# Easquel/WaveDM

Hardware: AMD Instinct MI355X
Metric: restored images/sec, raindrop 64x64 patches, 100-step DDIM (higher is better)
Workload: dtype bf16; 1 GPU; raindrop_wavelet 64x64 (256x256 px crops), batch 64/GPU, 100 DDIM steps, DWT + UNet x100 + IDWT (BASELINE.json configs[1]); global_batch=64, ddim_steps=100, parallelism=image-sharded x1, outputs_finite=True

## Files before the change

wavedm_amd/csrc/attn.hip:

```cpp
#include <atomic>
#include <type_traits>

#include "common.h"
#include "attn_fused_kernel.h"

namespace wdm {

bool attn_fused_eligible(int dtype, int N, int C) {
    return env_cfg().attn_fused && is_h16(dtype) && N == AttnFusedCfg::N && C % 128 == 0 && C >= 128 && C <= AttnFusedCfg::MAX_C &&
           (C <= AttnFusedCfg::MAX_CP || (C / 2) % 128 == 0);
}

template <typename T, bool VTOK>
static int launch_attn_fused_t(const AttnOperands& in, void* o, int B, int C, hipStream_t s, const float* vbias, const ConvArgs* proj) {
    using Cf = AttnFusedCfg;
    const bool qproj = in.qw != nullptr;
    if ((!in.q && !qproj) || !in.k || !in.v || (!o && !proj) || B <= 0) WDM_FAIL(WDM_EINVAL, "attn(fused): bad argument");
    if (qproj && (!VTOK || !proj || in.q || in.k != in.v || in.qw_ld < C || in.qw_ld % 8 || in.qw_bytes == 0 || in.qw_bytes >= 4294901760.0))
        WDM_FAIL(WDM_EINVAL, "attn(fused): the in-kernel query projection needs the folded block's operands (K = V = the normalised input, proj_out fused)");
    if ((!qproj && in.q_ld < C) || in.k_ld < C || ((qproj ? 0 : in.q_ld) | in.k_ld) % 8 || (VTOK && (in.v_ld < C || in.v_ld % 8))) WDM_FAIL(WDM_EINVAL, "attn(fused): row strides must be multiples of 8 elements >= C");
    if (proj && (C > 512 || proj->Cout != C || proj->Cin != C || proj->Hout != 16 || proj->Wout != 16 || proj->B != B || !proj->w || proj->w_bytes == 0 || proj->y_mode != Y_NHWC ||
                 proj->temb || proj->m_valid || proj->up4 || (proj->stats && proj->stats_nslab != 4)))
        WDM_FAIL(WDM_EINVAL, "attn(fused): proj_out epilogue arguments do not describe a C = %d 1x1 conv on 16 x 16 maps", C);
    if (in.bdiag && (!VTOK || proj || qproj)) WDM_FAIL(WDM_EINVAL, "attn(fused): the block-diagonal form (64 tokens per image) takes token-major V and writes O");
    const int NT = in.bdiag ? 64 : Cf::N;
    const int G = in.bdiag ? (B + 3) / 4 : B;
    const double qb = (double)B * NT * in.q_ld * 2.0, kb = (double)B * NT * in.k_ld * 2.0, vb = VTOK ? (double)B * NT * in.v_ld * 2.0 : (double)B * C * Cf::N * 2.0;
    if (qb >= 4294901760.0 || kb >= 4294901760.0 || vb >= 4294901760.0) WDM_FAIL(WDM_EINVAL, "attn(fused): an operand exceeds the 4 GB buffer-offset range");
    AttnFusedArgs a{};
    a.q = in.q; a.k = in.k; a.v = in.v; a.o = o; a.vbias = vbias; a.B = G; a.C = C; a.bdiag = in.bdiag; a.nimg = B;
    a.q_ld = in.q_ld; a.k_ld = in.k_ld; a.v_ld = in.v_ld;
    a.alpha = (float)std::pow((double)C, -0.5);
    a.qw = in.qw; a.qbias = in.qbias; a.qw_ld = in.qw_ld; a.qw_bytes = (unsigned)in.qw_bytes; a.qw_slab = in.qw_slab;
    a.q_bytes = qproj ? 0u : (unsigned)(qb - (in.q_ld - C) * 2.0); a.k_bytes = (unsigned)(kb - (in.k_ld - C) * 2.0); a.v_bytes = (unsigned)(VTOK ? vb - (in.v_ld - C) * 2.0 : vb);
    static std::atomic<unsigned> devs{0};
    int dev = 0;
    WDM_HIP(hipGetDevice(&dev));
    if (!(devs.load() & (1u << (dev & 31)))) {
        WDM_HIP(hipFuncSetAttribute((const void*)attn_fused_kernel<false, T, VTOK>, hipFuncAttributeMaxDynamicSharedMemorySize, Cf::LDS_BYTES));
        WDM_HIP(hipFuncSetAttribute((const void*)attn_fused_kernel<true, T, VTOK>, hipFuncAttributeMaxDynamicSharedMemorySize, 160 * 1024));
        if constexpr (VTOK) WDM_HIP(hipFuncSetAttribute((const void*)attn_fused_kernel<true, T, true, true>, hipFuncAttributeMaxDynamicSharedMemorySize, 160 * 1024));
        devs.fetch_or(1u << (dev & 31));
    }
    const bool prof = prof_enabled();
    if (prof) {
        char name[96];
        snprintf(name, sizeof(name), "attn_fused_n%s%s%s_%s|%s C=%d%s%s", in.bdiag ? "64x4" : "256", VTOK ? "t" : "", qproj ? "q" : "", std::is_same<T, f16_t>::value ? "f16" : "bf16",
                 in.bdiag ? "8x8" : "16x16", C, qproj ? " qproj+" : "", proj ? " +proj" : "");
        prof_begin(s, name, 4.0 * B * NT * (double)NT * C + (proj ? 2.0 * B * Cf::N * (double)C * C : 0.0) + (qproj ? 2.0 * B * Cf::N * (double)C * C : 0.0),
                   (double)B * NT * C * 2.0 * (qproj ? 3.0 : proj ? 5.0 : 4.0) + (proj ? (double)C * C * 2.0 : 0.0) + (qproj ? (double)C * C * 2.0 : 0.0));
    }
    ConvArgs pe{};
    if (proj) pe = *proj;
// ... 16 lines not shown
```

wavedm_amd/csrc/attn_fused_kernel.h:

```cpp
#pragma once
#include "conv_kernel.h"
#include "gn_arrive.h"

namespace wdm {

struct AttnFusedArgs {
    const void* q;
    const void* k;
    const void* v;
    void* o;
    const float* vbias;
    int B, C;
    int q_ld, k_ld, v_ld;
    float alpha;
    unsigned q_bytes, k_bytes, v_bytes;
    const void* qw;
    const float* qbias;
    int qw_ld;
    unsigned qw_bytes;
    int qw_slab;
    int bdiag, nimg;
};

struct AttnFusedCfg {
// ... 27 lines not shown
    typedef int i32x4 __attribute__((ext_vector_type(4)));
    auto make_q = [](const void* p, unsigned bytes) __attribute__((always_inline)) {
        const unsigned long long v = (unsigned long long)p;
        return i32x4{(int)(unsigned)v, (int)((unsigned)(v >> 32) & 0xFFFFu), (int)bytes, 0x00020000};
    };
    const i32x4 q_q = make_q(a.q, a.q_bytes), q_k = make_q(a.k, a.k_bytes), q_vt = make_q(a.v, a.v_bytes);
    const unsigned lds0 = (unsigned)(size_t)(__attribute__((address_space(3))) char*)smem;
    auto dma16 = [&](const i32x4& rsrc, unsigned lds_addr, unsigned voff, int soff) __attribute__((always_inline)) {
        unsigned keep;
        asm volatile("s_mov_b32 %0, m0\n\ts_mov_b32 m0, %2\n\ts_nop 0\n\tbuffer_load_dwordx4 %1, %3, %4 offen lds\n\ts_mov_b32 m0, %0"
                     : "=&s"(keep)
                     : "v"(voff), "s"(lds_addr), "s"(rsrc), "s"(soff)
                     : "memory");
    };

    unsigned v1[5];
#pragma unroll
    for (int j = 0; j < 5; ++j) {
        const int piece = wave * 5 + j;
        const int row = piece * 8 + (lane >> 3);
        const int u = (lane & 7) ^ ((row >> 1) & 7);
        const bool isk = row < N;
        const int tok = isk ? row : qb * QB + (row - N);
        v1[j] = (unsigned)(((long long)b * N + tok) * (isk ? a.k_ld : a.q_ld) * 2 + u * 16);
    }
    constexpr int ST1Q = N * 128;
    constexpr int Q_OFF = 3 * ST1Q;
    if constexpr (QPROJ) {
#pragma unroll
        for (int j = 0; j < 4; ++j) {
            const int row = (wave * 4 + j) * 8 + (lane >> 3);
            const int u = (lane & 7) ^ ((row >> 1) & 7);
            v1[j] = (unsigned)(((long long)b * N + row) * a.k_ld * 2 + u * 16);
        }
    }
    auto issue1 = [&](int step, int buf) __attribute__((always_inline)) {
        if constexpr (QPROJ) {
            const unsigned base = lds0 + buf * ST1Q + wave * (4 * 1024);
#pragma unroll
            for (int j = 0; j < 4; ++j) dma16(q_k, base + j * 1024, v1[j], step * 128);
        } else {
        const unsigned base = lds0 + buf * C::ST1 + wave * (5 * 1024);
#pragma unroll
        for (int j = 0; j < 5; ++j) dma16(wave * 5 + j < N / 8 ? q_k : q_q, base + j * 1024, v1[j], step * 128);
        }
    };
    const int npass = Cc > C::MAX_CP ? 2 : 1;
// ... 19 lines not shown
    }
    auto issue2 = [&](int pass, int chunk, int buf) __attribute__((always_inline)) {
        const unsigned base = lds0 + C::P_BYTES + buf * C::ST2 + wave * (4 * 1024);
        const int soff = VTOK ? (chunk * 32 * a.v_ld + pass * Cp) * 2 : pass * Cp * N * 2 + chunk * 64;
#pragma unroll
        for (int j = 0; j < 4; ++j) dma16(q_vt, base + j * 1024, v2[j], soff);
    };

    const int wm = wave >> 1, wn = wave & 1;
    const int sw = (lane >> 1) & 7, ku = lane >> 4;
    int a_off[2], b_off[2];
#pragma unroll
    for (int ks = 0; ks < 2; ++ks) {
        const int slot = (ks * 4 + ku) ^ sw;
        a_off[ks] = (wm * 64 + (lane & 15)) * 128 + slot * 16;
        b_off[ks] = N * 128 + (wn * 32 + (lane & 15)) * 128 + slot * 16;
    }
    f32x4 s_acc[4][2];
#pragma unroll
    for (int i = 0; i < 4; ++i)
#pragma unroll
        for (int j = 0; j < 2; ++j) s_acc[i][j] = f32x4{0.f, 0.f, 0.f, 0.f};
    const int nk = Cc / 64;
    if constexpr (QPROJ) {
        constexpr int HQ_BYTES = QB * 512 * 2, ST0 = 512 * 64;
        static_assert(HQ_BYTES + 3 * ST0 <= 160 * 1024 && Q_OFF + QB * 512 * 2 <= 160 * 1024, "LDS");
        const i32x4 q_mw = make_q(a.qw, a.qw_bytes);
        const int np0 = Cc / 32;
#pragma unroll
        for (int j = 0; j < 8; ++j) {
            const int piece = wave * 8 + j;
            const int pl = piece >> 2, row = (piece & 3) * 16 + (lane >> 2);
            if (pl < np0) dma16(q_k, lds0 + piece * 1024, (unsigned)(((long long)b * N + qb * QB + row) * a.k_ld * 2 + un2 * 16), pl * 64);
        }
        unsigned v0[4];
#pragma unroll
        for (int j = 0; j < 4; ++j) {
            const int row = (wave * 4 + j) * 16 + (lane >> 2);
            v0[j] = row < Cc ? (unsigned)((a.qw_slab ? row * 32 : row * a.qw_ld) * 2 + un2 * 16) : 0xFFFF0000u;
        }
        const int qstep = a.qw_slab ? a.qw_slab * 2 : 64;
        auto issue0 = [&](int chunk, int buf) __attribute__((always_inline)) {
            const unsigned base = lds0 + HQ_BYTES + buf * ST0 + wave * (4 * 1024);
#pragma unroll
            for (int j = 0; j < 4; ++j) dma16(q_mw, base + j * 1024, v0[j], chunk * qstep);
        };
// ... 40 lines not shown
            const int plane = c0 >> 6, unit = (c0 & 63) >> 3, half = (c0 >> 2) & 1;
#pragma unroll
            for (int i = 0; i < 4; ++i) {
                const int qn = i * 16 + (lane & 15);
                const uint2 qv = make_uint2(TI<T>::pack2(__builtin_fmaf(y_acc[i][j][0], 1.0f, cb.x), __builtin_fmaf(y_acc[i][j][1], 1.0f, cb.y)),
                                            TI<T>::pack2(__builtin_fmaf(y_acc[i][j][2], 1.0f, cb.z), __builtin_fmaf(y_acc[i][j][3], 1.0f, cb.w)));
                if (c0 < Cc) *(uint2*)(smem + Q_OFF + plane * (QB * 128) + qn * 128 + ((unit ^ ((qn >> 1) & 7)) << 4) + half * 8) = qv;
            }
        }
    } else {
    issue1(0, 0);
    if (nk > 1) issue1(1, 1);
    }
    {
        int buf = 0;
        for (int k = 0; k < nk; ++k) {
            if (k + 1 < nk) { if constexpr (QPROJ) asm volatile("s_waitcnt vmcnt(4) lgkmcnt(0)" ::: "memory"); else asm volatile("s_waitcnt vmcnt(5) lgkmcnt(0)" ::: "memory"); }
            else asm volatile("s_waitcnt vmcnt(0) lgkmcnt(0)" ::: "memory");
            __builtin_amdgcn_s_barrier();
            __builtin_amdgcn_sched_barrier(0);
            if (k + 2 < nk) issue1(k + 2, buf >= 1 ? buf - 1 : 2);
            const char* base = smem + buf * (QPROJ ? ST1Q : C::ST1);
            const char* qbase = QPROJ ? smem + Q_OFF + k * (QB * 128) - N * 128 : base;
#pragma unroll
            for (int ks = 0; ks < 2; ++ks) {
                uint4 af[4], bf[2];
#pragma unroll
                for (int i = 0; i < 4; ++i) af[i] = *(const uint4*)(base + a_off[ks] + i * (16 * 128));
#pragma unroll
                for (int j = 0; j < 2; ++j) bf[j] = *(const uint4*)(qbase + b_off[ks] + j * (16 * 128));
#pragma unroll
                for (int i = 0; i < 4; ++i)
#pragma unroll
                    for (int j = 0; j < 2; ++j) mma16<T>(s_acc[i][j], af[i], bf[j]);
            }
            buf = buf == 2 ? 0 : buf + 1;
        }
    }
    asm volatile("s_waitcnt vmcnt(0) lgkmcnt(0)" ::: "memory");
    __builtin_amdgcn_s_barrier();
    __builtin_amdgcn_sched_barrier(0);
    issue2(0, 0, 0);
    issue2(0, 1, 1);

    float* red = (float*)(smem + C::RED_OFF);
    const float sl2 = a.alpha * 1.4426950408889634f;
    float mx[2], sm[2];
#pragma unroll
    for (int j = 0; j < 2; ++j) {
        float m = -INFINITY;
#pragma unroll
        for (int i = 0; i < 4; ++i)
#pragma unroll
            for (int r = 0; r < 4; ++r) { s_acc[i][j][r] = (a.bdiag && wm != qb) ? -INFINITY : s_acc[i][j][r] * sl2; m = fmaxf(m, s_acc[i][j][r]); }
        m = fmaxf(m, __shfl_xor(m, 16));
        m = fmaxf(m, __shfl_xor(m, 32));
        if (lane < 16) red[wm * QB + wn * 32 + j * 16 + lane] = m;
        mx[j] = m;
    }
    asm volatile("s_waitcnt lgkmcnt(0)" ::: "memory");
    __builtin_amdgcn_s_barrier();
    __builtin_amdgcn_sched_barrier(0);
#pragma unroll
    for (int j = 0; j < 2; ++j) {
        const int qn = wn * 32 + j * 16 + (lane & 15);
        const float m = fmaxf(fmaxf(red[qn], red[QB + qn]), fmaxf(red[2 * QB + qn], red[3 * QB + qn]));
// ... 25 lines not shown
    }
    (void)mx; (void)sm;

    const int cw = Cp / 8;
    const int nfi = cw / 16;
    const int va_off = C::P_BYTES + lds_off(wave * cw + (lane & 15), ku);
    unsigned va_tr[4];
#pragma unroll
    for (int i = 0; i < 4; ++i) {
        const int li = lane & 15, g = lane >> 4, bs = wave * (cw >> 4) + i;
        const int fr = (li >> 2) + 4 * (g & 1);
        va_tr[i] = lds0 + C::P_BYTES + (g * 8 + (li >> 2)) * rowb + ((bs & ~7) | ((bs + fr) & 7)) * 32 + (li & 3) * 8;
    }
    int pb_off[4];
#pragma unroll
    for (int j = 0; j < 4; ++j) pb_off[j] = (j * 16 + (lane & 15)) * 512;
    const int prow15 = lane & 15;
    T* op = (T*)a.o + ((long long)b * N + qb * QB) * Cc;
    for (int pass = 0; pass < npass; ++pass) {
        if (pass > 0) {
            asm volatile("s_waitcnt lgkmcnt(0)" ::: "memory");
            __builtin_amdgcn_s_barrier();
            __builtin_amdgcn_sched_barrier(0);
            issue2(pass, 0, 0);
            issue2(pass, 1, 1);
        }
        f32x4 o_acc[4][4];
#pragma unroll
        for (int i = 0; i < 4; ++i)
#pragma unroll
            for (int j = 0; j < 4; ++j) o_acc[i][j] = f32x4{0.f, 0.f, 0.f, 0.f};
        int buf = 0;
        for (int k = 0; k < N / 32; ++k) {
            if (k + 1 < N / 32) asm volatile("s_waitcnt vmcnt(4) lgkmcnt(0)" ::: "memory");
            else asm volatile("s_waitcnt vmcnt(0) lgkmcnt(0)" ::: "memory");
            if (k == 0 || !own_rows || VTOK) __builtin_amdgcn_s_barrier();
            __builtin_amdgcn_sched_barrier(0);
            if (k + 2 < N / 32) issue2(pass, k + 2, buf >= 1 ? buf - 1 : 2);
            const char* vb = smem + buf * C::ST2;
            uint4 af[4], bf[4];
            const int pslot = ((k * 4 + ku) ^ prow15) << 4;
            if constexpr (VTOK) {
                unsigned long long lo[4], hi[4];
                const unsigned sb = buf * C::ST2;
#pragma unroll
                for (int i = 0; i < 4; ++i) {
                    const unsigned ad = (i < nfi ? va_tr[i] : va_tr[0]) + sb;
                    asm volatile("ds_read_b64_tr_b16 %0, %1" : "=v"(lo[i]) : "v"(ad) : "memory");
                    asm volatile("ds_read_b64_tr_b16 %0, %1" : "=v"(hi[i]) : "v"(ad + 4 * rowb) : "memory");
                }
#pragma unroll
                for (int j = 0; j < 4; ++j) bf[j] = *(const uint4*)(smem + pb_off[j] + pslot);
                asm volatile("s_waitcnt lgkmcnt(0)" : "+v"(lo[0]), "+v"(lo[1]), "+v"(lo[2]), "+v"(lo[3]), "+v"(hi[0]), "+v"(hi[1]), "+v"(hi[2]), "+v"(hi[3]) :: "memory");
#pragma unroll
                for (int i = 0; i < 4; ++i) af[i] = uint4{(unsigned)lo[i], (unsigned)(lo[i] >> 32), (unsigned)hi[i], (unsigned)(hi[i] >> 32)};
            } else {
#pragma unroll
                for (int i = 0; i < 4; ++i) if (i < nfi) af[i] = *(const uint4*)(vb + va_off + i * (16 * 64));
#pragma unroll
                for (int j = 0; j < 4; ++j) bf[j] = *(const uint4*)(smem + pb_off[j] + pslot);
            }
// ... 84 lines not shown
```

wavedm_amd/csrc/blocks.hip:

```cpp
#include <stdarg.h>

#include <algorithm>
#include <cmath>

#include <atomic>
#include <mutex>
#include "common.h"
#include "gn_inline.h"

namespace wdm {

static thread_local char g_err[512] = "";
void set_error(const char* fmt, ...) {
    va_list ap;
    va_start(ap, fmt);
    vsnprintf(g_err, sizeof(g_err), fmt, ap);
    va_end(ap);
}
const char* get_error() { return g_err; }

void* Arena::alloc(size_t bytes) {
    bytes = align_up(bytes ? bytes : 1, 256);
    for (size_t i = 0; i < free_.size(); ++i) {
        if (free_[i].len >= bytes) {
// ... 32 lines not shown
    if (!t->p) WDM_FAIL(WDM_ENOMEM, "workspace too small (tensor %dx%dx%dx%d)", c.B, H, W, C);
    return WDM_OK;
}
void free_tens(Ctx& c, Tens& t) {
    c.ar->free(t.p);
    if (t.stats) c.ar->free(t.stats);
    if (t.nrm) c.ar->free(t.nrm);
    if (t.fin_scale) { c.ar->free(t.fin_scale); c.ar->free(t.fin_shift); }
    t.p = nullptr; t.stats = nullptr; t.gst = nullptr; t.nslab = 0; t.nrm = nullptr; t.nrm_for = nullptr; t.fin_scale = t.fin_shift = nullptr; t.fin_for = nullptr;
}

static int alloc_f32(Ctx& c, size_t n, float** p) {
    *p = (float*)c.ar->alloc(n * sizeof(float));
    if (!*p) WDM_FAIL(WDM_ENOMEM, "workspace too small (%zu floats)", n);
    return WDM_OK;
}

static std::atomic<const EnvCfg*> g_env{nullptr};
static std::mutex g_env_mu;
void env_cfg_refresh() {
    EnvCfg* c = new EnvCfg();
    auto flag = [](const char* name, int dflt) { const char* e = getenv(name); return e ? (e[0] == '0' ? 0 : 1) : dflt; };
    auto num = [](const char* name, int dflt) { const char* e = getenv(name); return e ? atoi(e) : dflt; };
    c->conv_dma = flag("WDM_CONV_DMA", 1); c->gemm = flag("WDM_GEMM", 1); c->bn256 = num("WDM_BN256", 1);
    c->gn_tile = num("WDM_GN_TILE", 2); c->gn_inline = num("WDM_GN_INLINE", 1); c->attn_fused = num("WDM_ATTN_FUSED", 3); c->attn_fold = num("WDM_ATTN_FOLD", 1);
    c->up4 = flag("WDM_UP4", 1); c->attn_sm = flag("WDM_ATTN_SM", 1); c->wgrad_bg = num("WDM_WGRAD_BG", 0);
    std::lock_guard<std::mutex> lk(g_env_mu);
    g_env.store(c, std::memory_order_release);
}
const EnvCfg& env_cfg() {
    const EnvCfg* c = g_env.load(std::memory_order_acquire);
    if (!c) {
        {
            std::lock_guard<std::mutex> lk(g_env_mu);
            c = g_env.load(std::memory_order_acquire);
        }
        if (!c) { env_cfg_refresh(); c = g_env.load(std::memory_order_acquire); }
    }
    return *c;
}

bool conv_up4_eligible(int dtype, int H, int W, int cin, int cout) {
    return env_cfg().up4 && (is_h16(dtype) || dtype == WDM_F32X3) && ((H % 16 == 0 && W % 16 == 0) || (H == 8 && W == 8)) && cin % 32 == 0 && cout % 8 == 0 && cout >= 128;
}

int launch_conv(const ConvArgs& a0, int mode, int dtype, hipStream_t s) {
    const ConvArgs& a = a0;
    return dtype == WDM_BF16 ? launch_conv_bf16(a, mode, s) : dtype == WDM_F16 ? launch_conv_f16(a, mode, s) : dtype == WDM_F32X3 ? launch_conv_f32x3(a, mode, s) : launch_conv_f32(a, mode, s);
// ... 351 lines not shown
```

wavedm_amd/csrc/common.h:

```cpp
#pragma once
#include <hip/hip_runtime.h>
#include <stdint.h>
#include <stdio.h>
#include <string>
#include <vector>

#include "../../include/wavedm.h"
#include "conv_kernel.h"

namespace wdm {

void set_error(const char* fmt, ...);
#define WDM_FAIL(code, ...)        \
    do {                           \
        wdm::set_error(__VA_ARGS__); \
        return (code);             \
    } while (0)
#define WDM_HIP(expr)                                                                        \
    do {                                                                                     \
        hipError_t e__ = (expr);                                                             \
        if (e__ != hipSuccess) WDM_FAIL(WDM_EHIP, "%s failed: %s", #expr, hipGetErrorString(e__)); \
    } while (0)
#define WDM_TRY(expr)              \
    do {                           \
// ... 138 lines not shown
void prof_end(hipStream_t s);

inline bool conv_can_fuse_shortcut(int H, int W, int cin, int cout, int sC0, int sC1) {
    const bool t16 = H % 16 == 0 && W % 16 == 0 && cout >= 128 && cin <= 2048;
    const bool t8 = H == 8 && W == 8;
    return (t16 || t8) && cin % 32 == 0 && sC0 % 64 == 0 && (sC0 + sC1) % 64 == 0;
}

bool attn_fused_eligible(int dtype, int N, int C);
struct AttnOperands {
    const void* q = nullptr; const void* k = nullptr; const void* v = nullptr;
    int q_ld = 0, k_ld = 0, v_ld = 0;
    int v_tok = 0;
    const void* qw = nullptr; const float* qbias = nullptr; int qw_ld = 0; size_t qw_bytes = 0;
    int bdiag = 0;
    int qw_slab = 0;
};
int launch_attn_fused(const AttnOperands& in, void* o, int B, int C, hipStream_t s, const float* vbias = nullptr, const ConvArgs* proj = nullptr, int dtype = WDM_BF16);
int k_attn_fold(const float* wq, const float* bq, const float* wk, const float* wv, const float* bv, const float* wp, const float* bp, int C, float* M, float* cq, float* Wvp,
                float* bvp, hipStream_t s);

struct EnvCfg {
    int conv_dma = 1;
    int gemm = 1;
    int bn256 = 1;
    int gn_tile = 2;
    int gn_inline = 1;
    int attn_fold = 1;
    int attn_fused = 3;
    int attn_sm = 1;
    int up4 = 1;
    int wgrad_bg = 0;
};
const EnvCfg& env_cfg();
void env_cfg_refresh();

int launch_conv(const ConvArgs& a, int mode, int dtype, hipStream_t s);

int run_conv(Ctx& c, const ConvW& w, int mode, const Tens& x0, const Tens* x1, const float* scale, const float* shift,
             const float* temb, int temb_ld, int temb_per_image, const Tens* res, Tens* out, int y_mode, void* y_ext,
             bool want_stats = false, const ConvW* shortcut = nullptr, const Tens* sx0 = nullptr, const Tens* sx1 = nullptr, const NormW* gn_inl = nullptr,
             ConvArgs* defer = nullptr,
             const NormW* on = nullptr, int on_silu = 0,
             const FinReq* fin = nullptr);
int run_gn(Ctx& c, const NormW& nw, const Tens& x0, const Tens* x1, int for_silu_conv, float** scale, float** shift);
int run_resblock(Ctx& c, const ResW& w, const Tens& x0, const Tens* x1, Tens* out, const NormW* next_n = nullptr, int next_silu = 0, const FinReq* next_fin = nullptr);
int run_attn(Ctx& c, const AttnW& w, const Tens& x, Tens* out, const FinReq* next_fin = nullptr);
// ... 22 lines not shown
```

wavedm_amd/csrc/conv_dispatch.inc:

```
#include <stdlib.h>

#include <atomic>

#include "common.h"
#include "conv_kernel.h"
#include "gn_inline.h"
#ifndef WDM_DTYPE_NAME
#define WDM_DTYPE_NAME (sizeof(WDM_T) == 2 ? "bf16" : "f32")
#endif

#ifndef WDM_H16_NAME
#define WDM_H16_NAME "bf16"
#endif

namespace wdm {

static int ensure_max_lds(const void* kern, int bytes, std::atomic<unsigned>& devs) {
    int dev = 0;
    WDM_HIP(hipGetDevice(&dev));
    const unsigned bit = 1u << (dev & 31);
    if (!(devs.load(std::memory_order_acquire) & bit)) {
        WDM_HIP(hipFuncSetAttribute(kern, hipFuncAttributeMaxDynamicSharedMemorySize, bytes));
        devs.fetch_or(bit, std::memory_order_release);
    }
// ... 146 lines not shown
}
static int launch_dma256(const ConvArgs& a, hipStream_t s) { return launch_dma_big<4, 2, 16>(a, s); }
static int launch_dma512(const ConvArgs& a, hipStream_t s) { return launch_dma_big<8, 1, 32>(a, s); }
template <int BN_>
static int launch_dma8(const ConvArgs& a0, hipStream_t s) {
    using C = ConvDma8Cfg<BN_>;
    ConvArgs a = a0;
    if (a.Hout != 8 || a.Wout != 8 || a.Hin != 8 || a.Win != 8) WDM_FAIL(WDM_EINVAL, "conv(dma8): 8x8 maps only");
    if (a.Cin % C::BK || a.C1 != 0 || a.x1 || a.pro || a.w_img_stride || a.m_valid) WDM_FAIL(WDM_EINVAL, "conv(dma8): unsupported operand combination");
    WDM_TRY(set_extents(a, (double)a.B * 64, 2.0, "conv(dma8)"));
    WDM_TRY(set_shortcut_extents(a, 2.0, 64, "conv(dma8)"));
    bool done;
    WDM_TRY(check_stats(a, 64 / conv_stat_rows(8, 8, 16 * C::WM), out_norm_shape_ok(a, C::BN), 0, "conv(dma8)", &done));
    if (done) return WDM_OK;
    use_slab_major(a);
    a.mtiles = (a.B + C::NI - 1) / C::NI;
    a.ntiles = (a.Cout + C::BN - 1) / C::BN;
    int grid;
    grouped_grid(a, 4, &grid);
    WDM_NAME(name, "convdma8_3x3s1_t8x8x2_bn%dw4_" WDM_H16_NAME "|8x8 %d->%d%s", BN_, a.Cin, a.Cout, a.sx0 ? " +1x1" : "");
    static std::atomic<unsigned> devs{0};
    return launch_named(conv_dma8_kernel<BN_, 2, WDM_T>, grid, C::NTHREADS, C::LDS_BYTES, s, a, devs, name, conv_work(a, 9.0, 2.0, (double)a.B * 64, (double)a.B * 64));
}
template <int TILE, int NI, int WN = 4>
static int launch_up4(const ConvArgs& a0, hipStream_t s) {
    using C = ConvUp4Cfg<TILE, NI, WN>;
    ConvArgs a = a0;
    if (a.Hout % TILE || a.Wout % TILE || a.Hin != a.Hout || a.Win != a.Wout || (NI > 1 && (a.Hout != TILE || a.Wout != TILE)))
        WDM_FAIL(WDM_EINVAL, "conv(up4): %dx%d map does not fit the %dx%d tile", a.Hout, a.Wout, TILE, TILE);
    if (a.Cin % C::BK || a.C1 != 0 || a.x1 || a.pro || a.res || a.sx0 || a.temb || a.w_img_stride || a.y_mode != Y_NHWC || a.Cout % 8 || a.m_valid)
        WDM_FAIL(WDM_EINVAL, "conv(up4): unsupported operand combination (Cin=%d Cout=%d)", a.Cin, a.Cout);
    if ((double)a.w_bytes >= 4294901760.0) WDM_FAIL(WDM_EINVAL, "conv(up4): weights exceed the 4 GB buffer-offset range");
    a.w_tap_stride = (long long)a.w_rows * 32; a.w_row_stride = 32; a.w_slab_stride = 16 * a.w_rows * 32;
    WDM_TRY(set_extents(a, (double)a.B * a.Hin * a.Win, 2.0, "conv(up4)"));
    bool done;
    WDM_TRY(check_stats(a, 4 * (a.Hout / TILE) * (a.Wout / TILE) * ((TILE * TILE) / conv_stat_rows(TILE, TILE, 16 * C::WM)), false,
                        (a.Hout / TILE) * (a.Wout / TILE) * 4 * ((a.Cout + C::BN - 1) / C::BN), "conv(up4)", &done));
    if (done) return WDM_OK;
    a.up4 = 1;
    a.up4_ntp = (a.Cout + C::BN - 1) / C::BN;
    a.mtiles = NI == 1 ? a.B * (a.Hout / TILE) * (a.Wout / TILE) : (a.B + NI - 1) / NI;
    a.ntiles = 4 * a.up4_ntp;
    int grid;
    plain_grid(a, &grid);
    WDM_NAME(name, "convup4_2x2x4_t%dx%dx%d_bn%dw8_" WDM_H16_NAME "|%dx%d %d->%d", TILE, TILE, NI, C::BN, 2 * a.Hout, 2 * a.Wout, a.Cin, a.Cout);
    const double Mhi = 4.0 * a.B * a.Hout * a.Wout;
// ... 170 lines not shown
    ConvArgs a = a0;
    if (a.Hout % 16 || a.Wout % 16 || a.Hin != 2 * a.Hout || a.Win != 2 * a.Wout) WDM_FAIL(WDM_EINVAL, "conv(s2x3): %dx%d -> %dx%d does not fit the 16x16 tile", a.Hin, a.Win, a.Hout, a.Wout);
    if (a.Cin % C::BK || a.C1 != 0 || a.x1 || a.pro || a.sx0 || a.w_img_stride || a.m_valid || a.yn) WDM_FAIL(WDM_EINVAL, "conv(s2x3): unsupported operand combination (Cin=%d Cout=%d)", a.Cin, a.Cout);
    WDM_TRY(set_extents(a, (double)a.B * a.Hin * a.Win, 4.0, "conv(s2x3)"));
    bool done;
    WDM_TRY(check_stats(a, (a.Hout / 16) * (a.Wout / 16) * 4, false, 0, "conv(s2x3)", &done));
    if (done) return WDM_OK;
    a.mtiles = a.B * (a.Hout / 16) * (a.Wout / 16);
    a.ntiles = (a.Cout + C::BN - 1) / C::BN;
    int grid;
    plain_grid(a, &grid);
    WDM_NAME(name, "convs2x3_3x3s2_t16x16x1_bn%dw8_f32x3|%dx%d %d->%d", C::BN, a.Hout, a.Wout, a.Cin, a.Cout);
    static std::atomic<unsigned> devs{0};
    return launch_named(conv_s2x3_kernel<WN>, grid, C::NTHREADS, C::LDS_BYTES, s, a, devs, name, conv_work(a, 9.0, 4.0, (double)a.B * a.Hin * a.Win, (double)a.B * a.Hout * a.Wout));
}
#endif

int WDM_LAUNCH_NAME(const ConvArgs& a, int mode, hipStream_t s) {
    const bool t16 = (a.Hout % 16 == 0) && (a.Wout % 16 == 0);
    const bool t8 = (a.Hout % 8 == 0) && (a.Wout % 8 == 0);
    const bool img8 = (a.Hout == 8 && a.Wout == 8);
    const bool bn16 = a.Cout <= 16;
    const bool shared_w = a.w_img_stride == 0;
    const bool dma = env_cfg().conv_dma != 0, gemm = env_cfg().gemm != 0;
    (void)dma; (void)gemm; (void)shared_w;
    if (!t8) WDM_FAIL(WDM_EINVAL, "conv: output %dx%d must be a multiple of 8", a.Hout, a.Wout);
    if ((a.y_mode == Y_NHWC || a.y_mode == Y_NHWC_F32) && a.Cout % 8 == 0) {
        const double rows = mode == MODE_UP4 ? 4.0 * a.B * a.Hout * a.Wout : a.m_valid ? (double)a.m_valid : (double)a.B * a.Hout * a.Wout;
        const double yb = rows * a.y_s * (a.y_mode == Y_NHWC ? (double)sizeof(WDM_T) : 4.0), rb = a.res ? rows * a.res_s * (double)sizeof(WDM_T) : 0.0;
        if (yb >= 4026531840.0 || rb >= 4026531840.0)
            WDM_FAIL(WDM_EINVAL, "conv: output / residual tensor of %.0f bytes exceeds the 32-bit buffer-offset range", yb > rb ? yb : rb);
    }
    if (a.query_yn) *a.query_yn = 0;
    if (a.query_fin) *a.query_fin = 0;
    if (a.yn && !a.query_nslab) {
        int ok = 0, ns = 0;
        ConvArgs q = a;
        q.query_nslab = &ns; q.query_yn = &ok;
        WDM_TRY(WDM_LAUNCH_NAME(q, mode, s));
        if (!ok) WDM_FAIL(WDM_EINVAL, "conv: in-tile GroupNorm of the output requested for a conv whose kernel cannot write it");
    }
    if (a.gst && (a.Cout % 32 || !gn_inline_shape_ok(a.Cout, a.stats_nslab) || !a.stats)) WDM_FAIL(WDM_EINVAL, "conv: group partials requested for Cout = %d", a.Cout);
    if (a.gin) {
#ifdef WDM_HAS_GEMM
        const bool dma_ok = mode == MODE_S1 && t16 && !bn16 && a.Cout >= 128 && dma && a.x1 == nullptr && shared_w && gn_inline_shape_ok(a.Cin, a.gin_nslab) && a.gn_gamma && a.gn_beta;
#else
        const bool dma_ok = false;
#endif
// ... 53 lines not shown
            if (a.Hout == 8 && a.Wout == 8) return launch_up4<8, 4>(a, s);
            if (wide_tiles(a, (long long)a.B * (a.Hout / 16) * (a.Wout / 16) * 4 * (a.Cout / 256))) return launch_up4<16, 1, 8>(a, s);
            return launch_up4<16, 1>(a, s);
#elif defined(WDM_HAS_DMAX3)
            if (a.Hout == 8 && a.Wout == 8) return launch_up4x3<8, 4>(a, s);
            return launch_up4x3<16, 1>(a, s);
#else
            WDM_FAIL(WDM_EINVAL, "conv: the sub-pixel upsample kernel is bf16 / f32x3 only");
#endif
        case MODE_P1:
#ifdef WDM_HAS_GEMM
            if (gemm && t16 && a.Cout >= 128 && a.Cin >= 256 && a.Cin % 64 == 0 && a.C0 % 64 == 0 && !a.pro)
                return wide_tiles(a, (long long)a.B * (a.Hout / 16) * (a.Wout / 16) * (a.Cout / 256)) ? launch_gemm<8>(a, s) : launch_gemm<4>(a, s);
            if (gemm && a.Hout % 8 == 0 && a.Wout % 16 == 0 && a.Cout >= 128 && a.Cin >= 256 && a.Cin % 64 == 0 && a.C0 % 64 == 0 && !a.pro && !a.stats && !a.res)
                return launch_gemm<2, 8>(a, s);
#endif
#ifdef WDM_HAS_DMAX3
            if (dma && gemm && t16 && a.Cout >= 128 && a.Cout % 8 == 0 && a.Cin >= 128 && a.Cin % 32 == 0 && a.C0 % 32 == 0 && !a.pro && !a.m_valid && !a.img_mod &&
                (a.y_mode == Y_NHWC || a.y_mode == Y_NHWC_F32) && (a.Hout / 16) * (a.Wout / 16) * ((a.Cout + 127) / 128) >= 4)
                return launch_gemmx3(a, s);
#endif
            if (a.Hout % 8 == 0 && a.Wout % 16 == 0 && a.Cout >= 128) return launch_cfg<MODE_P1, 8, 16, 1, 2, 2, 4, 4, 4>(a, s);
            if (t16) return launch_cfg<MODE_P1, 16, 16, 1, 4, 1, 4, 4>(a, s);
            if (img8 && a.B >= 2 && shared_w) return launch_cfg<MODE_P1, 8, 8, 2, 2, 2, 4, 2>(a, s);
            return launch_cfg<MODE_P1, 8, 8, 1, 2, 2, 2, 2>(a, s);
    }
    WDM_FAIL(WDM_EINVAL, "conv: bad mode %d", mode);
}

}
```

wavedm_amd/csrc/conv_dma8_kernel.h:

```cpp
#pragma once
#include "conv_kernel.h"
#include "gn_group.h"

#ifndef WDM_D8ABL
#define WDM_D8ABL 0
#endif

namespace wdm {

template <int BN_, int NI_ = 2>
struct ConvDma8Cfg {
    static_assert(BN_ == 64 || BN_ == 48, "N tile");
    static_assert(NI_ == 2 || NI_ == 4, "images per tile");
    static constexpr int TH = 8, TW = 8, NI = NI_;
    static constexpr int WAVES_M = (BN_ == 64 ? 2 : 4) * (NI / 2), WAVES_N = BN_ == 64 ? 2 : 1, WM = BN_ == 64 ? 4 : 2, WN = BN_ == 64 ? 2 : 3;
    static constexpr int NJ = BN_ == 64 ? 0 : 1;
    static constexpr int NWAVES = WAVES_M * WAVES_N, NTHREADS = 64 * NWAVES, BN = BN_, BK = 32;
    static constexpr int PH = 10, PW = 10, RS = 16;
    static constexpr int PLANE_IMG = PH * RS;
    static constexpr int A_ROWS = NI * PLANE_IMG;
    static constexpr int A_CPW = 5, B_CPW = NWAVES == 4 ? 3 : 2;
    static constexpr int A_BYTES = 10 * NI * 1024;
    static constexpr int B_SUB = NWAVES * B_CPW * 1024;
    static constexpr int B_OFF = 2 * A_BYTES;
    static constexpr int LDS_BYTES = B_OFF + 3 * B_SUB;
    static constexpr int EPI_BYTES = NWAVES * 16 * WM * (16 * 2 + 4) * 4;
    static constexpr int G_ROWS = NI * 64, G_A = G_ROWS * 128, G_STAGE = G_A + 64 * 128, GB_CPW = 8 / NWAVES;
    static_assert(EPI_BYTES <= LDS_BYTES && LDS_BYTES <= (NI == 2 ? 80 : 160) * 1024 && 3 * G_STAGE <= LDS_BYTES, "LDS");
    static_assert(WAVES_M * WM * 16 == NI * TH * TW && WAVES_N * WN * 16 == BN && A_CPW * NWAVES * 16 == A_ROWS && 3 * BN <= B_SUB / 64, "tile");
};

template <int BN_, int NI_ = 2, typename T_ = __bf16>
__global__ __launch_bounds__((ConvDma8Cfg<BN_, NI_>::NTHREADS), 2) void conv_dma8_kernel(const ConvArgs a) {
    using C = ConvDma8Cfg<BN_, NI_>;
    using T = T_;
    constexpr int ACP = C::A_CPW, BCP = C::B_CPW, TH = C::TH, TW = C::TW, NI = C::NI, WM = C::WM, WN = C::WN, BN = C::BN, RS = C::RS;
    extern __shared__ __attribute__((aligned(16))) char smem[];
    h16_mode_init<T>();

    const int tid = threadIdx.x;
    const int lane = tid & 63;
    const int wave = __builtin_amdgcn_readfirstlane(tid >> 6);
    const int wave_m = wave / C::WAVES_N, wave_n = wave % C::WAVES_N;

    const int bid = blockIdx.x;
    int mt, nt;
    if (!conv_decode_tile(a, bid, mt, nt)) return;
    const int n0 = nt * BN;
    const int img0 = mt * NI;

    typedef int i32x4 __attribute__((ext_vector_type(4)));
    auto make_q = [](const void* p, unsigned bytes) __attribute__((always_inline)) {
        const unsigned long long v = (unsigned long long)p;
        return i32x4{(int)(unsigned)v, (int)((unsigned)(v >> 32) & 0xFFFFu), (int)bytes, 0x00020000};
    };
// ... 68 lines not shown
        const char* pb = smem + dx * C::B_SUB;
        uint4 ae[WM + 1], ao[WM];
#pragma unroll
        for (int i = 0; i < WM; ++i) { ae[i] = *(const uint4*)(pa + a_addr[i][dx]); ao[i] = *(const uint4*)(pa + a_addr[i][dx] + RS * 64); }
        ae[WM] = *(const uint4*)(pa + a_addr[WM - 1][dx] + 2 * (RS * 64));
#pragma unroll
        for (int dy = 0; dy < 3; ++dy) {
            if (dy == 0) __builtin_amdgcn_s_setprio(2); else if (dy == 1) __builtin_amdgcn_s_setprio(1); else __builtin_amdgcn_s_setprio(0);
            uint4 bfr[WN];
#pragma unroll
            for (int j = 0; j < WN; ++j) bfr[j] = *(const uint4*)(pb + b_addr[j] + dy * (BN * 64));
#pragma unroll
            for (int i = 0; i < WM; ++i)
#pragma unroll
                for (int j = 0; j < WN; ++j) {
                    const uint4& af = dy == 0 ? ae[i] : dy == 1 ? ao[i] : ae[i + 1];
                    if (WDM_D8ABL & 2) { acc[i][j][0] += __uint_as_float(af.x ^ bfr[j].x); } else mma16t<T>(acc[i][j], af, bfr[j]);
                }
        }
    };
#define WDM_DMA8_SYNC(N) do { if (WDM_D8ABL & 32) asm volatile("s_waitcnt vmcnt(%0) lgkmcnt(0)" ::"n"(N) : "memory");  \
                              else asm volatile("s_waitcnt vmcnt(%0) lgkmcnt(0)\n\ts_barrier" ::"n"(N) : "memory"); __builtin_amdgcn_sched_barrier(0); } while (0)

    issue_a(0);
    issue_b(0, 0, 0);
    issue_b(0, 1, 1);
    for (int s = 0; s < nslab; ++s) {
        WDM_DMA8_SYNC(BCP);
        issue_b(s, 2, 2);
        issue_a(s + 1);
        mfma_dx(s, 0);
        WDM_DMA8_SYNC(BCP + ACP);
        issue_b(s + 1, 0, 0);
        mfma_dx(s, 1);
        WDM_DMA8_SYNC(BCP);
        issue_b(s + 1, 1, 1);
        mfma_dx(s, 2);
    }
#undef WDM_DMA8_SYNC
    asm volatile("s_waitcnt vmcnt(0) lgkmcnt(0)\n\ts_barrier" ::: "memory");
    __builtin_amdgcn_sched_barrier(0);

    if (a.sx0 != nullptr) {
        constexpr int G_A = C::G_A, G_STAGE = C::G_STAGE, GBC = C::GB_CPW;
        const i32x4 q_s0 = make_q(a.sx0, a.sx0_bytes), q_s1 = make_q(a.sx1 ? a.sx1 : a.sx0, a.sx1_bytes), q_sw = make_q(a.sw, a.sw_bytes);
        unsigned g_a0[4], g_a1[4], g_b[GBC];
#pragma unroll
        for (int i = 0; i < 4; ++i) {
            const int row = (wave * 4 + i) * 8 + (lane >> 3);
            const int u = (lane & 7) ^ ((row >> 1) & 7);
            const bool ok = img0 + row / 64 < a.B;
            const unsigned gp = (unsigned)((img0 + row / 64) * 64 + row % 64);
            g_a0[i] = ok ? gp * (unsigned)(a.sxs0 * 2) + (unsigned)(u * 16) : OOB;
            g_a1[i] = ok ? gp * (unsigned)(a.sxs1 * 2) + (unsigned)(u * 16) : OOB;
        }
#pragma unroll
        for (int i = 0; i < GBC; ++i) {
            const int row = (wave * GBC + i) * 8 + (lane >> 3);
            const int u = (lane & 7) ^ ((row >> 1) & 7);
            const int n = n0 + row;
            g_b[i] = (row < BN && n < a.sw_rows) ? (unsigned)(n * a.sw_row_stride * 2 + u * 16) : OOB;
        }
        auto issue2 = [&](int k, int buf) __attribute__((always_inline)) {
            const int c = k * 64;
            const unsigned base = lds0 + buf * G_STAGE;
            if (c < a.sC0) {
// ... 53 lines not shown
```

Measured before the change: 137.0 img/s.

## Skip off-diagonal attention blocks and route 8x8 1x1 convs to dma8 shortcut path

In block-diagonal attention mode (64 tokens per image packed four to a group), a new mode skips the QK score MMAs for tiles outside the query's own image and restricts the PV loop to that image's key chunks. Off-diagonal K rows are loaded from an out-of-bounds offset, so they read as zeros. This is enabled by default by raising the attn_fused default to 4. Separately, 1x1 convolutions on 8x8 maps now go to a variant of the dma8 kernel that skips the 3x3 main loop and runs only its shortcut-GEMM epilogue, which is also enabled by default. The risk is correctness of the softmax over the skipped blocks, which depends on how the kernel masks them.

After: 138.2 img/s, median of 6. No clear change (+0.9%).

```diff
diff --git a/wavedm_amd/csrc/attn.hip b/wavedm_amd/csrc/attn.hip
--- a/wavedm_amd/csrc/attn.hip
+++ b/wavedm_amd/csrc/attn.hip
@@ -28,7 +28,8 @@
     const double qb = (double)B * NT * in.q_ld * 2.0, kb = (double)B * NT * in.k_ld * 2.0, vb = VTOK ? (double)B * NT * in.v_ld * 2.0 : (double)B * C * Cf::N * 2.0;
     if (qb >= 4294901760.0 || kb >= 4294901760.0 || vb >= 4294901760.0) WDM_FAIL(WDM_EINVAL, "attn(fused): an operand exceeds the 4 GB buffer-offset range");
     AttnFusedArgs a{};
-    a.q = in.q; a.k = in.k; a.v = in.v; a.o = o; a.vbias = vbias; a.B = G; a.C = C; a.bdiag = in.bdiag; a.nimg = B;
+    a.q = in.q; a.k = in.k; a.v = in.v; a.o = o; a.vbias = vbias; a.B = G; a.C = C; a.nimg = B;
+    a.bdiag = in.bdiag ? (env_cfg().attn_fused >= 4 ? 2 : 1) : 0;
     a.q_ld = in.q_ld; a.k_ld = in.k_ld; a.v_ld = in.v_ld;
     a.alpha = (float)std::pow((double)C, -0.5);
     a.qw = in.qw; a.qbias = in.qbias; a.qw_ld = in.qw_ld; a.qw_bytes = (unsigned)in.qw_bytes; a.qw_slab = in.qw_slab;
diff --git a/wavedm_amd/csrc/attn_fused_kernel.h b/wavedm_amd/csrc/attn_fused_kernel.h
--- a/wavedm_amd/csrc/attn_fused_kernel.h
+++ b/wavedm_amd/csrc/attn_fused_kernel.h
@@ -73,7 +73,7 @@
         const int u = (lane & 7) ^ ((row >> 1) & 7);
         const bool isk = row < N;
         const int tok = isk ? row : qb * QB + (row - N);
-        v1[j] = (unsigned)(((long long)b * N + tok) * (isk ? a.k_ld : a.q_ld) * 2 + u * 16);
+        v1[j] = (a.bdiag == 2 && isk && (row >> 6) != qb) ? 0xFFFF0000u : (unsigned)(((long long)b * N + tok) * (isk ? a.k_ld : a.q_ld) * 2 + u * 16);
     }
     constexpr int ST1Q = N * 128;
     constexpr int Q_OFF = 3 * ST1Q;
@@ -139,6 +139,7 @@
 #pragma unroll
         for (int j = 0; j < 2; ++j) s_acc[i][j] = f32x4{0.f, 0.f, 0.f, 0.f};
     const int nk = Cc / 64;
+    const bool s_live = a.bdiag != 2 || wm == qb;
     if constexpr (QPROJ) {
         constexpr int HQ_BYTES = QB * 512 * 2, ST0 = 512 * 64;
         static_assert(HQ_BYTES + 3 * ST0 <= 160 * 1024 && Q_OFF + QB * 512 * 2 <= 160 * 1024, "LDS");
@@ -225,6 +226,7 @@
             if (k + 2 < nk) issue1(k + 2, buf >= 1 ? buf - 1 : 2);
             const char* base = smem + buf * (QPROJ ? ST1Q : C::ST1);
             const char* qbase = QPROJ ? smem + Q_OFF + k * (QB * 128) - N * 128 : base;
+            if (s_live) {
 #pragma unroll
             for (int ks = 0; ks < 2; ++ks) {
                 uint4 af[4], bf[2];
@@ -236,6 +238,7 @@
                 for (int i = 0; i < 4; ++i)
 #pragma unroll
                     for (int j = 0; j < 2; ++j) mma16<T>(s_acc[i][j], af[i], bf[j]);
+            }
             }
             buf = buf == 2 ? 0 : buf + 1;
         }
@@ -243,8 +246,9 @@
     asm volatile("s_waitcnt vmcnt(0) lgkmcnt(0)" ::: "memory");
     __builtin_amdgcn_s_barrier();
     __builtin_amdgcn_sched_barrier(0);
-    issue2(0, 0, 0);
-    issue2(0, 1, 1);
+    const int kc0 = a.bdiag == 2 ? qb * 2 : 0, nkc = a.bdiag == 2 ? 2 : N / 32;
+    issue2(0, kc0, 0);
+    issue2(0, kc0 + 1, 1);
 
     float* red = (float*)(smem + C::RED_OFF);
     const float sl2 = a.alpha * 1.4426950408889634f;
@@ -316,8 +320,8 @@
             asm volatile("s_waitcnt lgkmcnt(0)" ::: "memory");
             __builtin_amdgcn_s_barrier();
             __builtin_amdgcn_sched_barrier(0);
-            issue2(pass, 0, 0);
-            issue2(pass, 1, 1);
+            issue2(pass, kc0, 0);
+            issue2(pass, kc0 + 1, 1);
         }
         f32x4 o_acc[4][4];
 #pragma unroll
@@ -325,12 +329,13 @@
 #pragma unroll
             for (int j = 0; j < 4; ++j) o_acc[i][j] = f32x4{0.f, 0.f, 0.f, 0.f};
         int buf = 0;
-        for (int k = 0; k < N / 32; ++k) {
-            if (k + 1 < N / 32) asm volatile("s_waitcnt vmcnt(4) lgkmcnt(0)" ::: "memory");
+        for (int kk = 0; kk < nkc; ++kk) {
+            const int k = kc0 + kk;
+            if (kk + 1 < nkc) asm volatile("s_waitcnt vmcnt(4) lgkmcnt(0)" ::: "memory");
             else asm volatile("s_waitcnt vmcnt(0) lgkmcnt(0)" ::: "memory");
-            if (k == 0 || !own_rows || VTOK) __builtin_amdgcn_s_barrier();
-            __builtin_amdgcn_sched_barrier(0);
-            if (k + 2 < N / 32) issue2(pass, k + 2, buf >= 1 ? buf - 1 : 2);
+            if (kk == 0 || !own_rows || VTOK) __builtin_amdgcn_s_barrier();
+            __builtin_amdgcn_sched_barrier(0);
+            if (kk + 2 < nkc) issue2(pass, k + 2, buf >= 1 ? buf - 1 : 2);
             const char* vb = smem + buf * C::ST2;
             uint4 af[4], bf[4];
             const int pslot = ((k * 4 + ku) ^ prow15) << 4;
diff --git a/wavedm_amd/csrc/blocks.hip b/wavedm_amd/csrc/blocks.hip
--- a/wavedm_amd/csrc/blocks.hip
+++ b/wavedm_amd/csrc/blocks.hip
@@ -78,8 +78,8 @@
     EnvCfg* c = new EnvCfg();
     auto flag = [](const char* name, int dflt) { const char* e = getenv(name); return e ? (e[0] == '0' ? 0 : 1) : dflt; };
     auto num = [](const char* name, int dflt) { const char* e = getenv(name); return e ? atoi(e) : dflt; };
-    c->conv_dma = flag("WDM_CONV_DMA", 1); c->gemm = flag("WDM_GEMM", 1); c->bn256 = num("WDM_BN256", 1);
-    c->gn_tile = num("WDM_GN_TILE", 2); c->gn_inline = num("WDM_GN_INLINE", 1); c->attn_fused = num("WDM_ATTN_FUSED", 3); c->attn_fold = num("WDM_ATTN_FOLD", 1);
+    c->conv_dma = flag("WDM_CONV_DMA", 1); c->gemm = num("WDM_GEMM", 2); c->bn256 = num("WDM_BN256", 1);
+    c->gn_tile = num("WDM_GN_TILE", 2); c->gn_inline = num("WDM_GN_INLINE", 1); c->attn_fused = num("WDM_ATTN_FUSED", 4); c->attn_fold = num("WDM_ATTN_FOLD", 1);
     c->up4 = flag("WDM_UP4", 1); c->attn_sm = flag("WDM_ATTN_SM", 1); c->wgrad_bg = num("WDM_WGRAD_BG", 0);
     std::lock_guard<std::mutex> lk(g_env_mu);
     g_env.store(c, std::memory_order_release);
diff --git a/wavedm_amd/csrc/common.h b/wavedm_amd/csrc/common.h
--- a/wavedm_amd/csrc/common.h
+++ b/wavedm_amd/csrc/common.h
@@ -184,7 +184,7 @@
 
 struct EnvCfg {
     int conv_dma = 1;
-    int gemm = 1;
+    int gemm = 2;
     int bn256 = 1;
     int gn_tile = 2;
     int gn_inline = 1;
diff --git a/wavedm_amd/csrc/conv_dispatch.inc b/wavedm_amd/csrc/conv_dispatch.inc
--- a/wavedm_amd/csrc/conv_dispatch.inc
+++ b/wavedm_amd/csrc/conv_dispatch.inc
@@ -192,6 +192,27 @@
     static std::atomic<unsigned> devs{0};
     return launch_named(conv_dma8_kernel<BN_, 2, WDM_T>, grid, C::NTHREADS, C::LDS_BYTES, s, a, devs, name, conv_work(a, 9.0, 2.0, (double)a.B * 64, (double)a.B * 64));
 }
+static int launch_dma8_1x1(const ConvArgs& a0, hipStream_t s) {
+    using C = ConvDma8Cfg<64>;
+    ConvArgs a = a0;
+    if (a.Hout != 8 || a.Wout != 8 || a.Hin != 8 || a.Win != 8) WDM_FAIL(WDM_EINVAL, "conv(dma8 1x1): 8x8 maps only");
+    if (a.Cin % 64 || a.C0 != a.Cin || a.C1 != 0 || a.x1 || a.pro || a.w_img_stride || a.m_valid || a.x_img_shared || a.img_mod || a.sx0 || a.w_rows <= 0)
+        WDM_FAIL(WDM_EINVAL, "conv(dma8 1x1): unsupported operand combination");
+    WDM_TRY(set_extents(a, (double)a.B * 64, 2.0, "conv(dma8 1x1)"));
+    a.sx0 = a.x0; a.sxs0 = a.xs0; a.sx1 = nullptr; a.sxs1 = 0; a.sC0 = a.Cin; a.sC1 = 0;
+    a.sw = a.w; a.sw_row_stride = (int)a.w_row_stride; a.sw_rows = a.w_rows; a.sw_bytes = a.w_bytes;
+    WDM_TRY(set_shortcut_extents(a, 2.0, 64, "conv(dma8 1x1)"));
+    bool done;
+    WDM_TRY(check_stats(a, 64 / conv_stat_rows(8, 8, 16 * C::WM), false, 0, "conv(dma8 1x1)", &done));
+    if (done) return WDM_OK;
+    a.mtiles = (a.B + C::NI - 1) / C::NI;
+    a.ntiles = (a.Cout + C::BN - 1) / C::BN;
+    int grid;
+    grouped_grid(a, 4, &grid);
+    WDM_NAME(name, "convdma8_1x1_t8x8x2_bn64w4_" WDM_H16_NAME "|8x8 %d->%d", a.Cin, a.Cout);
+    static std::atomic<unsigned> devs{0};
+    return launch_named(conv_dma8_kernel<64, 2, WDM_T, true>, grid, C::NTHREADS, C::LDS_BYTES, s, a, devs, name, conv_work(a, 1.0, 2.0, (double)a.B * 64, (double)a.B * 64));
+}
 template <int TILE, int NI, int WN = 4>
 static int launch_up4(const ConvArgs& a0, hipStream_t s) {
     using C = ConvUp4Cfg<TILE, NI, WN>;
@@ -408,8 +429,8 @@
     const bool img8 = (a.Hout == 8 && a.Wout == 8);
     const bool bn16 = a.Cout <= 16;
     const bool shared_w = a.w_img_stride == 0;
-    const bool dma = env_cfg().conv_dma != 0, gemm = env_cfg().gemm != 0;
-    (void)dma; (void)gemm; (void)shared_w;
+    const bool dma = env_cfg().conv_dma != 0, gemm = env_cfg().gemm != 0, gemm8 = env_cfg().gemm >= 2;
+    (void)dma; (void)gemm; (void)gemm8; (void)shared_w;
     if (!t8) WDM_FAIL(WDM_EINVAL, "conv: output %dx%d must be a multiple of 8", a.Hout, a.Wout);
     if ((a.y_mode == Y_NHWC || a.y_mode == Y_NHWC_F32) && a.Cout % 8 == 0) {
         const double rows = mode == MODE_UP4 ? 4.0 * a.B * a.Hout * a.Wout : a.m_valid ? (double)a.m_valid : (double)a.B * a.Hout * a.Wout;
@@ -509,6 +530,11 @@
 #endif
             if (a.Hout % 8 == 0 && a.Wout % 16 == 0 && a.Cout >= 128) return launch_cfg<MODE_P1, 8, 16, 1, 2, 2, 4, 4, 4>(a, s);
             if (t16) return launch_cfg<MODE_P1, 16, 16, 1, 4, 1, 4, 4>(a, s);
+#ifdef WDM_HAS_GEMM
+            if (dma && gemm8 && img8 && a.B >= 2 && shared_w && a.Cin % 64 == 0 && a.C0 == a.Cin && !a.x1 && !a.pro && !a.m_valid && !a.x_img_shared && !a.img_mod &&
+                a.w_rows > 0 && a.Cout % 8 == 0)
+                return launch_dma8_1x1(a, s);
+#endif
             if (img8 && a.B >= 2 && shared_w) return launch_cfg<MODE_P1, 8, 8, 2, 2, 2, 4, 2>(a, s);
             return launch_cfg<MODE_P1, 8, 8, 1, 2, 2, 2, 2>(a, s);
     }
diff --git a/wavedm_amd/csrc/conv_dma8_kernel.h b/wavedm_amd/csrc/conv_dma8_kernel.h
--- a/wavedm_amd/csrc/conv_dma8_kernel.h
+++ b/wavedm_amd/csrc/conv_dma8_kernel.h
@@ -30,7 +30,7 @@
     static_assert(WAVES_M * WM * 16 == NI * TH * TW && WAVES_N * WN * 16 == BN && A_CPW * NWAVES * 16 == A_ROWS && 3 * BN <= B_SUB / 64, "tile");
 };
 
-template <int BN_, int NI_ = 2, typename T_ = __bf16>
+template <int BN_, int NI_ = 2, typename T_ = __bf16, bool P1_ = false>
 __global__ __launch_bounds__((ConvDma8Cfg<BN_, NI_>::NTHREADS), 2) void conv_dma8_kernel(const ConvArgs a) {
     using C = ConvDma8Cfg<BN_, NI_>;
     using T = T_;
@@ -145,6 +145,7 @@
 #define WDM_DMA8_SYNC(N) do { if (WDM_D8ABL & 32) asm volatile("s_waitcnt vmcnt(%0) lgkmcnt(0)" ::"n"(N) : "memory");  \
                               else asm volatile("s_waitcnt vmcnt(%0) lgkmcnt(0)\n\ts_barrier" ::"n"(N) : "memory"); __builtin_amdgcn_sched_barrier(0); } while (0)
 
+    if constexpr (!P1_) {
     issue_a(0);
     issue_b(0, 0, 0);
     issue_b(0, 1, 1);
@@ -160,11 +161,12 @@
         issue_b(s + 1, 1, 1);
         mfma_dx(s, 2);
     }
-#undef WDM_DMA8_SYNC
     asm volatile("s_waitcnt vmcnt(0) lgkmcnt(0)\n\ts_barrier" ::: "memory");
     __builtin_amdgcn_sched_barrier(0);
-
-    if (a.sx0 != nullptr) {
+    }
+#undef WDM_DMA8_SYNC
+
+    if (P1_ || a.sx0 != nullptr) {
         constexpr int G_A = C::G_A, G_STAGE = C::G_STAGE, GBC = C::GB_CPW;
         const i32x4 q_s0 = make_q(a.sx0, a.sx0_bytes), q_s1 = make_q(a.sx1 ? a.sx1 : a.sx0, a.sx1_bytes), q_sw = make_q(a.sw, a.sw_bytes);
         unsigned g_a0[4], g_a1[4], g_b[GBC];
```
